# pbluc/avrecode-ms

Measured on AMD Instinct MI355X. Metric: H.264 bytes/s recompressed (CABAC re-encode of recorded bin streams, bit-exact vs CPU), higher is better.
Workload: dtype u32

## Files before the change

avrecode-ms_amd/csrc/avr_k1p.h:

```cpp
#pragma once
#include <stdint.h>

#include "avr_chunk.h"

#if defined(__HIPCC__)
#define AVR_HD __host__ __device__ inline
#else
#define AVR_HD inline
#endif

namespace avr {
namespace k1p {

#if defined(__HIP_DEVICE_COMPILE__)
#define AVR_PIN2(a, b) asm volatile("" : "+v"(a), "+v"(b))
#else
#define AVR_PIN2(a, b) ((void)0)
#endif

constexpr uint32_t kNone = 0xffffffffu;
constexpr uint32_t kMaxStretch = 16 * kChunk;
constexpr uint32_t kCodeBypass = 252;
constexpr uint32_t kCodePad = 252;

struct alignas(16) U4 { uint32_t x, y, z, w; };

AVR_HD int clz32(uint32_t x) {
#if defined(__HIP_DEVICE_COMPILE__)
    return __clz(x);
#else
    return x ? __builtin_clz(x) : 32;
#endif
}

AVR_HD uint32_t code_sym(uint32_t c) { return ((c >> 1) ^ c) & 1u; }
AVR_HD bool code_is_bypass(uint32_t c) { return (c >> 1) == 126u; }
AVR_HD bool code_is_boundary(uint32_t c) { return code_sym(c) && !code_is_bypass(c); }
AVR_HD uint32_t code_terminate(uint32_t b) { return 255u - b; }
AVR_HD uint32_t code_context(uint32_t s, uint32_t bin) { return s >= 126 ? 255u - ((bin ^ s) & 1u) : (s << 1) | bin; }

AVR_HD uint32_t post_lps_range(uint32_t row, uint32_t q, uint32_t *shift) {
    const uint32_t rl = (row >> (8 * q)) & 0xffu;
    const uint32_t sh = uint32_t(clz32(rl)) - 23;
    *shift = sh;
    return rl << sh;
}

struct CodeEntry { uint32_t row, meta; };
AVR_HD CodeEntry code_entry(uint32_t c, const uint32_t *rows ) {
    if (code_is_bypass(c)) return CodeEntry{0u, 0x100u | ((c & 1u) << 1)};
    return CodeEntry{rows[c >> 2], code_sym(c) * 3u};
}

AVR_HD int clz32_nz(uint32_t x) { return __builtin_clz(x); }
AVR_HD uint32_t lps_range(uint32_t row, uint32_t R) {
#if defined(__HIP_DEVICE_COMPILE__)
    return __builtin_amdgcn_perm(row, 0u, R >> 6);
#else
    return (row >> ((R >> 3) & 24)) & 0xffu;
#endif
}
AVR_HD uint32_t mul24(uint32_t a, uint32_t b) {
#if defined(__HIP_DEVICE_COMPILE__)
    return __umul24(a, b);
#else
    return a * b;
#endif
}
AVR_HD uint32_t step_range(const CodeEntry &e, uint32_t *R) {
    const uint32_t rl = lps_range(e.row, *R);
    const uint32_t rm = *R - rl;
    const uint32_t x = (e.meta & 1u) ? rl : rm;
    const uint32_t sh = uint32_t(clz32_nz(x)) - 23;
    *R = x << sh;
    return sh + (e.meta >> 8);
}

struct alignas(16) CodeEntryC { uint32_t row, side, k, adj; };
AVR_HD CodeEntryC code_entry_c(const CodeEntry &e) {
    const uint32_t sym = e.meta & 1u, adds = (e.meta >> 1) & 1u, byp = e.meta >> 8;
    return CodeEntryC{e.row, sym ? ~0u : 0u, adds ? (byp ? 1u : 2u) : 0u, byp - 23u};
}
AVR_HD uint32_t step_range_c(const CodeEntryC &e, uint32_t *R, uint32_t *v) {
    const uint32_t rl = lps_range(e.row, *R);
    const uint32_t rm = *R - rl;
    const uint32_t x = (rl & e.side) | (rm & ~e.side);
    const uint32_t lz = uint32_t(clz32_nz(x));
    *v = mul24(rm, e.k);
    *R = x << (lz - 23);
    return lz + e.adj;
}


struct Stretch {
    uint32_t first;
    uint32_t end;
    uint32_t t_exit[4];
    uint16_t r_exit[4];
    uint8_t exit_q;
    uint8_t too_long;
    uint8_t pad[2];
};

struct LinearCodes {
    const uint8_t *p;
    AVR_HD U4 load16(uint32_t i) const { return *reinterpret_cast<const U4 *>(p + i); }
    AVR_HD uint32_t byte(uint32_t i) const { return p[i]; }
};

template <class Src, class F>
AVR_HD void for_codes_in(const Src &src, uint32_t from, uint32_t n, F &&f) {
    for (uint32_t base = from & ~15u; base < n; base += 16) {
        const U4 v = src.load16(base);
        uint32_t w0 = v.x, w1 = v.y, w2 = v.z, w3 = v.w;
#if defined(__HIP_DEVICE_COMPILE__)
#pragma unroll 1
#endif
        for (uint32_t k = 0; k < 4; k++) {
            const uint32_t d = w0;
            w0 = w1; w1 = w2; w2 = w3;
            const uint32_t i = base + 4 * k;
            if (i + 0 - from < n - from && f(i + 0, d & 0xffu)) return;
            if (i + 1 - from < n - from && f(i + 1, (d >> 8) & 0xffu)) return;
            if (i + 2 - from < n - from && f(i + 2, (d >> 16) & 0xffu)) return;
            if (i + 3 - from < n - from && f(i + 3, d >> 24)) return;
        }
    }
}
template <class F>
AVR_HD void for_codes(const uint8_t *res, uint32_t from, uint32_t n, F &&f) { for_codes_in(LinearCodes{res}, from, n, f); }

template <class G, class G4>
AVR_HD void for_codes_all(const uint8_t *res, uint32_t from, uint32_t to, G &&g, G4 &&g4) {
    if (from >= to) return;
    auto group16 = [&](const U4 &v) {
        uint32_t w0 = v.x, w1 = v.y, w2 = v.z, w3 = v.w;
#if defined(__HIP_DEVICE_COMPILE__)
#pragma unroll 1
#endif
        for (uint32_t k = 0; k < 4; k++) {
            const uint32_t d = w0;
            w0 = w1; w1 = w2; w2 = w3;
            g4(d);
        }
    };
    const uint32_t head_end = ((from + 15) & ~15u) < to ? ((from + 15) & ~15u) : to;
    for_codes(res, from, head_end, [&](uint32_t, uint32_t c) { g(c); return false; });
    uint32_t base = head_end;
    for (; (base & 63) && base + 16 <= to; base += 16) group16(*reinterpret_cast<const U4 *>(res + base));
    if (base + 64 <= to) {
        const U4 *p = reinterpret_cast<const U4 *>(res + base);
        U4 v0 = p[0], v1 = p[1], v2 = p[2], v3 = p[3];
        for (; base + 64 <= to; base += 64) {
            const U4 *q = reinterpret_cast<const U4 *>(res + (base + 128 <= to ? base + 64 : base));
            const U4 n0 = q[0], n1 = q[1], n2 = q[2], n3 = q[3];
            group16(v0); group16(v1); group16(v2); group16(v3);
            v0 = n0; v1 = n1; v2 = n2; v3 = n3;
        }
    }
    for (; base + 16 <= to; base += 16) group16(*reinterpret_cast<const U4 *>(res + base));
    if (base < to) for_codes(res, base, to, [&](uint32_t, uint32_t c) { g(c); return false; });
}

AVR_HD void code_entries4(const CodeEntry *codes, uint32_t d, CodeEntry e[4]) {
    e[0] = codes[d & 0xffu]; e[1] = codes[(d >> 8) & 0xffu]; e[2] = codes[(d >> 16) & 0xffu]; e[3] = codes[d >> 24];
    AVR_PIN2(e[0].row, e[0].meta); AVR_PIN2(e[1].row, e[1].meta); AVR_PIN2(e[2].row, e[2].meta); AVR_PIN2(e[3].row, e[3].meta);
}
AVR_HD void code_entries4(const CodeEntryC *codes, uint32_t d, CodeEntryC e[4]) {
    e[0] = codes[d & 0xffu]; e[1] = codes[(d >> 8) & 0xffu]; e[2] = codes[(d >> 16) & 0xffu]; e[3] = codes[d >> 24];
    AVR_PIN2(e[0].row, e[0].side); AVR_PIN2(e[1].row, e[1].side); AVR_PIN2(e[2].row, e[2].side); AVR_PIN2(e[3].row, e[3].side);
}

AVR_HD void b1_stretch(const uint8_t *res, uint32_t n, uint32_t chunk, const CodeEntry *codes, uint32_t max_stretch,
                       Stretch *o) {
    const uint32_t lo = chunk_start(chunk), limit = chunk_start(chunk + 1);
    uint32_t R[4], T[4] = {0, 0, 0, 0};
    uint32_t i;
    o->too_long = 0;
    o->exit_q = 0;
    o->pad[0] = o->pad[1] = 0;
    if (chunk == 0) {
        o->first = 0;
        R[0] = R[1] = R[2] = R[3] = 510;
        i = 0;
    } else {
// ... 237 lines not shown
```

avrecode-ms_amd/csrc/avr_k1p.hip:

```cpp
#include <hip/hip_runtime.h>

#include <mutex>
#include <stdint.h>
#include <stdlib.h>
#include <type_traits>

#include "avr_coder.h"
#include "avr_internal.h"
#include "avr_k1p.h"
#include "avr_tables.h"

namespace avr {

static __device__ const CabacTables d_tables = make_cabac_tables();

using namespace k1p;

struct Plan {
    const uint16_t *recs;
    const uint64_t *rec_off;
    const uint32_t *n_bins;
    const uint64_t *res_off;
    const uint32_t *chunk_base, *chunk_slice;
    const uint32_t *blk_base, *blk_slice;
    const uint64_t *dig_off;
    uint32_t n_states;
    uint32_t ns_full;
    const uint16_t *table;
    const uint16_t *index;
    const uint8_t *recs8;
};
constexpr uint32_t kNotUsed = 0xffffu;

struct TileCodes {
    const uint8_t *base;
    uint32_t chunk0;
    __device__ __forceinline__ size_t at(uint32_t i) const {
        return group_at(chunk0 + chunk_of(i), bin_in_chunk(i) >> 4);
    }
    static __device__ __forceinline__ size_t group_at(uint32_t gc, uint32_t g) { return ((size_t(gc >> 6) * kChunkCodeGroups + g) * kTileChunks + (gc & 63u)) * 16; }
    __device__ __forceinline__ U4 load16(uint32_t i) const { return *reinterpret_cast<const U4 *>(base + at(i)); }
    __device__ __forceinline__ uint32_t byte(uint32_t i) const { return base[at(i) + (i & 15u)]; }
};


constexpr uint32_t kCensusBlocks = 32;
__global__ __launch_bounds__(256) void k_k1p_census(Plan p, uint32_t total_blocks, const int32_t *status, uint32_t *used, uint32_t stride) {
    __shared__ uint8_t flag[AVR_MAX_STATES];
    __shared__ uint32_t bm[32];
    for (uint32_t k = threadIdx.x; k < AVR_MAX_STATES / 4; k += 256) reinterpret_cast<uint32_t *>(flag)[k] = 0;
    if (threadIdx.x < 32) bm[threadIdx.x] = 0;
    __syncthreads();
    const uint32_t b = blockIdx.x * kCensusBlocks + (threadIdx.x >> 3), t = threadIdx.x & 7, nk = p.ns_full;
    if (b < total_blocks) {
        const uint32_t s = p.blk_slice[b];
        if (status[s] == AVR_SLICE_OK) {
            const uint32_t n = p.n_bins[s], i0 = (b - p.blk_base[s]) * kSortBlock;
            const uint32_t i1 = i0 + kSortBlock < n ? i0 + kSortBlock : n;
            const uint16_t *r = p.recs + p.rec_off[s];
            for (uint32_t l = b % stride; l < kSortBlock / 64; l += stride) {
                const uint32_t i = i0 + l * 64 + t * 8;
                if (i >= i1) continue;
                const uint4 v = *reinterpret_cast<const uint4 *>(r + i);
                const uint32_t w[4] = {v.x, v.y, v.z, v.w};
#pragma unroll
                for (uint32_t j = 0; j < 8; j++) {
                    const uint32_t sel = ((w[j >> 1] >> ((j & 1) * 16)) & 0xffffu) >> 1;
                    if (i + j < i1 && sel < nk) flag[sel] = 1;
                }
            }
        }
    }
    __syncthreads();
    {
        const uint32_t f = reinterpret_cast<const uint32_t *>(flag)[threadIdx.x];
        const uint32_t nib = (f & 1u) | ((f >> 7) & 2u) | ((f >> 14) & 4u) | ((f >> 21) & 8u);
        if (nib) atomicOr(&bm[threadIdx.x >> 3], nib << ((threadIdx.x & 7) * 4));
    }
    __syncthreads();
    if (threadIdx.x < 32) {
        const uint32_t mine = bm[threadIdx.x];
        if (mine & ~__hip_atomic_load(&used[threadIdx.x], __ATOMIC_RELAXED, __HIP_MEMORY_SCOPE_AGENT)) atomicOr(&used[threadIdx.x], mine);
    }
}

__global__ __launch_bounds__(256) void k_k1p_swap(int32_t *status, uint32_t n, int32_t a, int32_t b, int32_t c, int32_t d) {
    const uint32_t i = blockIdx.x * 256 + threadIdx.x;
    if (i >= n) return;
    const int32_t v = status[i];
    if (v == a) status[i] = b;
    else if (v == c) status[i] = d;
}

__global__ __launch_bounds__(AVR_MAX_STATES) void k_k1p_densemap(const uint32_t *used, uint16_t *table, uint16_t *index, uint32_t *n_dense) {
    __shared__ uint32_t sc[AVR_MAX_STATES];
    const uint32_t k = threadIdx.x;
    const uint32_t bit = (used[k >> 5] >> (k & 31)) & 1u;
    sc[k] = bit;
    __syncthreads();
    for (uint32_t d = 1; d < AVR_MAX_STATES; d <<= 1) {
        const uint32_t v = k >= d ? sc[k - d] : 0;
        __syncthreads();
        sc[k] += v;
        __syncthreads();
    }
    const uint32_t id = sc[k] - bit;
    table[k] = bit ? uint16_t(id) : uint16_t(kNotUsed);
    if (bit) index[id] = uint16_t(k);
    if (k >= sc[AVR_MAX_STATES - 1]) index[k] = uint16_t(kNotUsed);
    if (k == AVR_MAX_STATES - 1) *n_dense = sc[AVR_MAX_STATES - 1];
}

__global__ __launch_bounds__(256) void k_k1p_tn(uint8_t *tn) {
    const uint32_t i = blockIdx.x * 256 + threadIdx.x;
    if (i >= kTnBytes) return;
    const uint32_t n = 31 - __clz((i >> 7) + 1), j = i - ((128u << n) - 128u);
    uint32_t st = j >> n;
    for (uint32_t b = 0; b < n; b++) {
        const uint32_t nx = d_tables.packed[st][1], bin = (j >> b) & 1u;
        st = ((bin ^ st) & 1u) ? (nx >> 8) & 0xffu : nx & 0xffu;
    }
    tn[i] = uint8_t(st);
}

template <class F>
__device__ __forceinline__ void for_record_groups(const uint16_t *r, uint32_t i0, uint32_t i1, F &&f) {
    uint32_t i = i0;
    if (i + 32 <= i1) {
        const uint32_t last = i0 + ((i1 - i0) / 32u - 1u) * 32u;
        const U4 *q = reinterpret_cast<const U4 *>(r + i);
        U4 v0 = q[0], v1 = q[1], v2 = q[2], v3 = q[3];
        for (; i + 32 <= i1; i += 32) {
            const U4 *qn = reinterpret_cast<const U4 *>(r + (i + 32 <= last ? i + 32 : last));
            const U4 n0 = qn[0], n1 = qn[1], n2 = qn[2], n3 = qn[3];
            f(i, v0, std::false_type{}); f(i + 8, v1, std::false_type{}); f(i + 16, v2, std::false_type{}); f(i + 24, v3, std::false_type{});
            v0 = n0; v1 = n1; v2 = n2; v3 = n3;
        }
    }
    for (; i < i1; i += 8) f(i, *reinterpret_cast<const U4 *>(r + i), std::true_type{});
}

template <class F>
__device__ __forceinline__ void for_record_groups8(const uint8_t *r, uint32_t i0, uint32_t i1, F &&f) {
    uint32_t i = i0;
    if (i + 64 <= i1) {
        const uint32_t last = i0 + ((i1 - i0) / 64u - 1u) * 64u;
        const U4 *q = reinterpret_cast<const U4 *>(r + i);
        U4 v0 = q[0], v1 = q[1], v2 = q[2], v3 = q[3];
        for (; i + 64 <= i1; i += 64) {
            const U4 *qn = reinterpret_cast<const U4 *>(r + (i + 64 <= last ? i + 64 : last));
            const U4 n0 = qn[0], n1 = qn[1], n2 = qn[2], n3 = qn[3];
            f(i, v0, std::false_type{}); f(i + 16, v1, std::false_type{}); f(i + 32, v2, std::false_type{}); f(i + 48, v3, std::false_type{});
            v0 = n0; v1 = n1; v2 = n2; v3 = n3;
        }
    }
    for (; i < i1; i += 16) f(i, *reinterpret_cast<const U4 *>(r + i), std::true_type{});
}

template <class SelT, bool R8>
__global__ __launch_bounds__(512) void k_k1p_local(Plan p, uint32_t total_chunks, int32_t *status, uint32_t *lbits,
                                                   uint16_t *lend, uint32_t *n_retry) {
    extern __shared__ uint32_t local_lds[];
    constexpr uint32_t kSelTab = R8 ? 128 : 2048;
    __shared__ SelT sel_tab[kSelTab];
    const uint32_t nk = p.n_states, lane = threadIdx.x & 63, wv = threadIdx.x >> 6;
    const uint32_t cnt_rows = (nk + 5) / 2;
    const uint32_t wave_dwords = (kChunkBitDwords + 1 + cnt_rows) * 64;
    uint32_t *bits = local_lds + wv * wave_dwords;
    uint32_t *cnt = bits + (kChunkBitDwords + 1) * 64;
    for (uint32_t sel = threadIdx.x; sel < kSelTab; sel += blockDim.x) {
        uint32_t k;
        if (R8) k = sel < nk ? sel : sel == AVR_SEL8_TERMINATE ? nk : sel == AVR_SEL8_BYPASS ? nk + 1 : nk + 3;
        else if (sel < AVR_MAX_STATES) {
            const uint32_t d = p.table[sel];
            k = d < nk ? d : sel < p.ns_full ? nk + 2 : nk + 3;
        } else k = sel == AVR_SEL_TERMINATE ? nk : sel == AVR_SEL_BYPASS ? nk + 1 : nk + 3;
        sel_tab[sel] = SelT((k >> 1) * 256u | (k & 1u) * 16u);
    }
    for (uint32_t i = lane; i < wave_dwords; i += 64) bits[i] = 0;
    __syncthreads();
    const uint32_t gc0 = (blockIdx.x * (blockDim.x >> 6) + wv) * 64, gc = gc0 + lane;
    uint32_t i0 = 0, i1 = 0, n = 0, s = 0;
    bool mine = false;
    const uint16_t *r = p.recs;
    const uint8_t *r8 = p.recs8;
    uint32_t misaligned = 0;
    if (gc < total_chunks) {
        s = p.chunk_slice[gc];
        if (status[s] == AVR_SLICE_OK) {
            mine = true;
            n = p.n_bins[s];
            const ChunkSpan sp = chunk_span(gc - p.chunk_base[s], n);
            i1 = sp.i1; i0 = sp.i0 > i1 ? i1 : sp.i0;
            if (R8) {
                const uint64_t off = p.rec_off[s];
                misaligned = uint32_t(off & 15u);
                r8 = p.recs8 + (off & ~uint64_t(15));
            } else {
                r = p.recs + p.rec_off[s];
            }
        }
    }
    uint32_t *my_cnt = cnt + lane;
    uint32_t *my_bits = bits + lane;
    uint8_t *cnt_b = reinterpret_cast<uint8_t *>(my_cnt), *bits_b = reinterpret_cast<uint8_t *>(my_bits);
    auto for_groups = [&](auto &&f) { for_record_groups(r, i0, i1, f); };
    uint32_t high = 0;
    const uint32_t k_pad = nk + 1;
    const uint32_t e_pad = (k_pad >> 1) * 256u | (k_pad & 1u) * 16u;
    auto group8 = [&](uint32_t base, const U4 &v, auto masked, uint32_t e[16], uint32_t bin[16]) {
        const uint32_t w[4] = {v.x, v.y, v.z, v.w};
#pragma unroll
        for (uint32_t j = 0; j < 16; j++) {
            const uint32_t b = (w[j >> 2] >> (8 * (j & 3))) & 0xffu;
            e[j] = sel_tab[b >> 1];
            if (decltype(masked)::value) e[j] = base + j < i1 ? e[j] : e_pad;
            bin[j] = b & 1u;
        }
    };
    if (R8) for_record_groups8(r8, i0, i1, [&](uint32_t base, const U4 &v, auto masked) {
        uint32_t e[16], bin[16];
        group8(base, v, masked, e, bin);
#pragma unroll
        for (uint32_t j = 0; j < 16; j++)
            __hip_atomic_fetch_add(reinterpret_cast<uint32_t *>(cnt_b + (e[j] & ~255u)), 1u << (e[j] & 31u), __ATOMIC_RELAXED,
                                   __HIP_MEMORY_SCOPE_WORKGROUP);
    });
    else for_groups([&](uint32_t base, const U4 &v, auto masked) {
        const uint32_t w[4] = {v.x, v.y, v.z, v.w};
        high |= (w[0] | w[1]) | (w[2] | w[3]);
        uint32_t e[8];
#pragma unroll
        for (uint32_t j = 0; j < 8; j++) {
            e[j] = sel_tab[((w[j >> 1] >> ((j & 1) * 16)) >> 1) & 0x7ffu];
            if (decltype(masked)::value) e[j] = base + j < i1 ? e[j] : e_pad;
        }
#pragma unroll
        for (uint32_t j = 0; j < 8; j++)
            __hip_atomic_fetch_add(reinterpret_cast<uint32_t *>(cnt_b + (e[j] & ~255u)), 1u << (e[j] & 31u), __ATOMIC_RELAXED,
                                   __HIP_MEMORY_SCOPE_WORKGROUP);
    });
    auto count_of = [&](uint32_t k) { return (my_cnt[64 * (k >> 1)] >> (16 * (k & 1u))) & 0xffffu; };
    const uint32_t n_term = count_of(nk), n_missed = count_of(nk + 2), n_invalid = count_of(nk + 3) | (high & 0xf000f000u) | misaligned;
    uint32_t term_at = 0;
    {
        uint32_t run = 0;
        for (uint32_t j = 0; j < cnt_rows; j++) {
            const uint32_t c = my_cnt[64 * j], c0 = c & 0xffffu, c1 = c >> 16;
            const uint32_t s0 = 2 * j <= nk ? run : kChunk, s1 = 2 * j + 1 <= nk ? run + c0 : kChunk;
            if (2 * j == nk) term_at = s0;
            if (2 * j + 1 == nk) term_at = s1;
            my_cnt[64 * j] = s0 | s1 << 16;
            run += (2 * j <= nk ? c0 : 0u) + (2 * j + 1 <= nk ? c1 : 0u);
        }
    }
    if (R8) for_record_groups8(r8, i0, i1, [&](uint32_t base, const U4 &v, auto masked) {
        uint32_t e[16], bin[16], pos[16];
        group8(base, v, masked, e, bin);
#pragma unroll
        for (uint32_t j = 0; j < 16; j++)
            pos[j] = __hip_atomic_fetch_add(reinterpret_cast<uint32_t *>(cnt_b + (e[j] & ~255u)), 1u << (e[j] & 31u), __ATOMIC_RELAXED,
                                            __HIP_MEMORY_SCOPE_WORKGROUP);
#pragma unroll
        for (uint32_t j = 0; j < 16; j++) {
            const uint32_t at = (pos[j] >> (e[j] & 31u)) & kChunkPosMask;
            const uint32_t row = at >> 5 < kChunkBitDwords ? at >> 5 : kChunkSpareRow;
            __hip_atomic_fetch_or(reinterpret_cast<uint32_t *>(bits_b + row * 256u), bin[j] << (at & 31u), __ATOMIC_RELAXED,
                                  __HIP_MEMORY_SCOPE_WORKGROUP);
        }
    });
    else for_groups([&](uint32_t base, const U4 &v, auto masked) {
        const uint32_t w[4] = {v.x, v.y, v.z, v.w};
        uint32_t e[8], pos[8];
#pragma unroll
        for (uint32_t j = 0; j < 8; j++) {
            e[j] = sel_tab[((w[j >> 1] >> ((j & 1) * 16)) >> 1) & 0x7ffu];
            if (decltype(masked)::value) e[j] = base + j < i1 ? e[j] : e_pad;
        }
#pragma unroll
        for (uint32_t j = 0; j < 8; j++)
            pos[j] = __hip_atomic_fetch_add(reinterpret_cast<uint32_t *>(cnt_b + (e[j] & ~255u)), 1u << (e[j] & 31u), __ATOMIC_RELAXED,
                                            __HIP_MEMORY_SCOPE_WORKGROUP);
#pragma unroll
        for (uint32_t j = 0; j < 8; j++) {
            const uint32_t at = (pos[j] >> (e[j] & 31u)) & kChunkPosMask;
            const uint32_t row = at >> 5 < kChunkBitDwords ? at >> 5 : kChunkSpareRow;
            const uint32_t bin = (w[j >> 1] >> ((j & 1) * 16)) & 1u;
            __hip_atomic_fetch_or(reinterpret_cast<uint32_t *>(bits_b + row * 256u), bin << (at & 31u), __ATOMIC_RELAXED,
                                  __HIP_MEMORY_SCOPE_WORKGROUP);
        }
    });
    if (mine) {
        uint32_t ones = 0;
        for (uint32_t pos = term_at; pos < term_at + n_term;) {
            const uint32_t lo = pos & 31u, take = 32u - lo < term_at + n_term - pos ? 32u - lo : term_at + n_term - pos;
            const uint32_t mask = (take == 32u ? 0xffffffffu : (1u << take) - 1u) << lo;
            ones += __popc(my_bits[64 * (pos >> 5)] & mask);
            pos += take;
        }
        constexpr uint32_t kTerm1 = (AVR_SEL_TERMINATE << 1) | 1, kTerm1_8 = (AVR_SEL8_TERMINATE << 1) | 1;
        auto last_is_term1 = [&]() { return i1 == n && (R8 ? r8[misaligned + n - 1] == kTerm1_8 : r[n - 1] == kTerm1); };
        const bool bad_term = ones > 1u || (ones == 1u && !last_is_term1());
        if (n_invalid || bad_term) status[s] = AVR_SLICE_BAD_RECORD;
        else if (n_missed && atomicCAS(&status[s], AVR_SLICE_OK, AVR_SLICE_RETRY_CENSUS) == AVR_SLICE_OK) atomicAdd(n_retry, 1u);
    }
    {
        uint32_t *dst = lbits + size_t(gc0) * kChunkBitDwords;
        const uint32_t lim = gc0 < total_chunks ? (total_chunks - gc0 < 64 ? total_chunks - gc0 : 64) * kChunkBitDwords : 0;
        for (uint32_t f = lane; f < lim; f += 64) dst[f] = bits[64 * (f % kChunkBitDwords) + f / kChunkBitDwords];
    }
    if (nk) {
        uint16_t *dst = lend + size_t(gc0) * nk;
        const uint32_t lim = gc0 < total_chunks ? (total_chunks - gc0 < 64 ? total_chunks - gc0 : 64) * nk : 0;
        uint32_t ch = lane / nk, k = lane - ch * nk;
        const uint32_t dch = 64 / nk, dk = 64 - dch * nk;
        for (uint32_t f = lane; f < lim; f += 64) {
            dst[f] = uint16_t(cnt[64 * (k >> 1) + ch] >> (16 * (k & 1u)));
            ch += dch; k += dk;
            if (k >= nk) { k -= nk; ch++; }
        }
    }
}

constexpr uint32_t kChainLanes = 22, kChainWaves = 8;
__device__ __forceinline__ uint4 window(const uint32_t *bw, uint32_t pos) {
    const uint32_t wi = (pos >> 5) & (kChunkBitDwords - 1);
    return make_uint4(bw[wi], bw[wi + 1], bw[wi + 2], bw[wi + 3]);
}
__global__ __launch_bounds__(64 * kChainWaves) void k_k1p_ctxchain(Plan p, uint32_t n_slices, uint32_t groups, uint32_t chain_lanes, const int32_t *status,
                                                      const uint8_t *tng, const uint32_t *lbits, const uint16_t *lend,
                                                      const uint8_t *init_states, uint8_t *est, uint8_t *final_states) {
    __shared__ uint8_t tn[kTnBytes];
    for (uint32_t i = threadIdx.x; i < kTnBytes / 16; i += 64 * kChainWaves) reinterpret_cast<uint4 *>(tn)[i] = reinterpret_cast<const uint4 *>(tng)[i];
    __syncthreads();
    const uint32_t wave = blockIdx.x * kChainWaves + (threadIdx.x >> 6), lane = threadIdx.x & 63;
    const uint32_t nk = p.n_states, pair = wave * 64 + lane;
    const uint32_t s = groups ? wave / groups : pair / nk, k = groups ? (wave - s * groups) + lane * groups : pair - s * nk;
    if ((groups && lane >= chain_lanes) || s >= n_slices || status[s] != AVR_SLICE_OK || k >= nk) return;
    const uint32_t col = p.index ? p.index[k] : k, row4 = ((nk + 3) >> 2) << 2;
    if (col >= p.ns_full) return;
    uint32_t st = init_states[size_t(s) * p.ns_full + col] & 127u;
    const uint32_t c0 = p.chunk_base[s], nc = chunks_of(p.n_bins[s]);
    const uint16_t *le = lend + size_t(c0) * nk + k;
    const uint32_t *bw_ahead = lbits + size_t(c0) * kChunkBitDwords;
    const uint32_t *bw_cur = bw_ahead;
    uint8_t *eo = est + size_t(c0) * row4 + k;
    auto ends = [&]() {
        const uint32_t e1 = le[0], em = le[-1];
        le += nk;
        return make_uint2(k ? em : 0u, e1);
    };
    uint2 e0 = ends(), e1 = ends(), e2 = ends(), e3 = ends();
    uint4 w0 = window(bw_ahead, e0.x), w1 = window(bw_ahead + kChunkBitDwords, e1.x);
    bw_ahead += 2 * kChunkBitDwords;
    for (uint32_t c = 0; c < nc; c++) {
        const uint2 e4 = ends();
        const uint4 w2 = window(bw_ahead, e2.x);
        bw_ahead += kChunkBitDwords;
        *eo = uint8_t(st);
        eo += row4;
        uint32_t pos = e0.x;
        const uint32_t end = e0.y;
        uint32_t left = (end > pos && st < 126) ? end - pos : 0u;
        const uint32_t sh = pos & 31u;
        auto four = [&](uint32_t avail) {
#pragma unroll
            for (uint32_t i = 0; i < 4; i++) {
                if (i && !__any(left != 0)) break;
                const uint32_t n = left < 8u ? left : 8u;
                uint32_t off = (128u << n) - 128u + (avail & ((1u << n) - 1u));
                asm volatile("" : "+v"(off));
                st = tn[(st << n) + off];
                avail >>= 8;
                left -= n;
            }
        };
        four(__builtin_amdgcn_alignbit(w0.y, w0.x, sh));
        if (__any(left != 0)) {
            four(__builtin_amdgcn_alignbit(w0.z, w0.y, sh));
            if (__any(left != 0)) {
                pos += 64;
                uint32_t avail = __builtin_amdgcn_alignbit(w0.w, w0.z, sh);
                uint32_t have = 32;
                while (left) {
                    if (have == 0) {
                        const uint4 win = window(bw_cur, pos);
                        avail = __builtin_amdgcn_alignbit(win.y, win.x, pos & 31u);
                        have = 32;
                    }
                    const uint32_t n = left < 8u ? left : 8u;
                    uint32_t off = (128u << n) - 128u + (avail & ((1u << n) - 1u));
                    asm volatile("" : "+v"(off));
                    st = tn[(st << n) + off];
                    avail >>= 8;
                    left -= n; pos += n; have -= 8;
                }
            }
        }
        bw_cur += kChunkBitDwords;
        e0 = e1; e1 = e2; e2 = e3; e3 = e4;
        w0 = w1; w1 = w2;
    }
    if (final_states) final_states[size_t(s) * p.ns_full + col] = uint8_t(st);
}

constexpr uint32_t kSegWaves = 16;
constexpr uint32_t kChainWaveSlots = 8192;

template <int NS>
__device__ __forceinline__ void chain_step(const uint8_t *tn, const uint32_t *bw_cur, uint32_t pos, uint32_t end, const uint4 &w0, uint32_t (&st)[NS]) {
    uint32_t left = end > pos ? end - pos : 0u;
    const uint32_t sh = pos & 31u;
    auto four = [&](uint32_t avail) {
#pragma unroll
        for (uint32_t i = 0; i < 4; i++) {
            if (i && !__any(left != 0)) break;
            const uint32_t n = left < 8u ? left : 8u;
            uint32_t off = (128u << n) - 128u + (avail & ((1u << n) - 1u));
            asm volatile("" : "+v"(off));
#pragma unroll
            for (int q = 0; q < NS; q++) st[q] = tn[(st[q] << n) + off];
            avail >>= 8;
            left -= n;
        }
    };
    four(__builtin_amdgcn_alignbit(w0.y, w0.x, sh));
    if (__any(left != 0)) {
        four(__builtin_amdgcn_alignbit(w0.z, w0.y, sh));
        if (__any(left != 0)) {
            pos += 64;
            uint32_t avail = __builtin_amdgcn_alignbit(w0.w, w0.z, sh);
            uint32_t have = 32;
            while (left) {
                if (have == 0) {
                    const uint32_t wi = (pos >> 5) & (kChunkBitDwords - 1);
                    avail = __builtin_amdgcn_alignbit(bw_cur[wi + 1], bw_cur[wi], pos & 31u);
                    have = 32;
                }
                const uint32_t n = left < 8u ? left : 8u;
                uint32_t off = (128u << n) - 128u + (avail & ((1u << n) - 1u));
                asm volatile("" : "+v"(off));
#pragma unroll
                for (int q = 0; q < NS; q++) st[q] = tn[(st[q] << n) + off];
                avail >>= 8;
                left -= n; pos += n; have -= 8;
            }
        }
    }
}

struct ChainLane { uint32_t s, k, seg, c_begin, c_end, nc, col; };
__device__ __forceinline__ bool chain_lane(const Plan &p, uint32_t n_slices, uint32_t n_segs, const int32_t *status, ChainLane *o) {
    const uint32_t wave = blockIdx.x * kSegWaves + (threadIdx.x >> 6), lane = threadIdx.x & 63, nk = p.n_states;
    const uint32_t seg = wave % n_segs, pair = (wave / n_segs) * 64 + lane;
    const uint32_t s = pair / nk, k = pair - s * nk;
    if (s >= n_slices || status[s] != AVR_SLICE_OK) return false;
    const uint32_t col = p.index ? p.index[k] : k;
    if (col >= p.ns_full) return false;
    const uint32_t nc = chunks_of(p.n_bins[s]), seg_len = (nc + n_segs - 1) / n_segs;
    const uint32_t c_begin = seg * seg_len < nc ? seg * seg_len : nc, c_end = c_begin + seg_len < nc ? c_begin + seg_len : nc;
    *o = ChainLane{s, k, seg, c_begin, c_end, nc, col};
    return true;
}

__global__ __launch_bounds__(64 * kSegWaves) void k_k1p_chain_seg(Plan p, uint32_t n_slices, uint32_t n_segs, const int32_t *status,
                                                       const uint8_t *tng, const uint32_t *lbits, const uint16_t *lend, uint8_t *est, SegSummary *summ) {
    __shared__ uint8_t tn[kTnBytes];
    for (uint32_t i = threadIdx.x; i < kTnBytes / 16; i += 64 * kSegWaves) reinterpret_cast<uint4 *>(tn)[i] = reinterpret_cast<const uint4 *>(tng)[i];
    __syncthreads();
    ChainLane L;
    if (!chain_lane(p, n_slices, n_segs, status, &L)) return;
    const uint32_t nk = p.n_states, row4 = ((nk + 3) >> 2) << 2, k = L.k;
    const uint32_t c0 = p.chunk_base[L.s] + L.c_begin, n_ch = L.c_end - L.c_begin;
    const uint16_t *le = lend + size_t(c0) * nk + k;
    const uint32_t *bw_ahead = lbits + size_t(c0) * kChunkBitDwords, *bw_cur = bw_ahead;
    uint8_t *eo = est + size_t(c0) * row4 + k;
    auto ends = [&]() { const uint32_t e1 = le[0], em = le[-1]; le += nk; return make_uint2(k ? em : 0u, e1); };
    uint2 e0 = ends(), e1 = ends(), e2 = ends(), e3 = ends();
    uint4 w0 = window(bw_ahead, e0.x), w1 = window(bw_ahead + kChunkBitDwords, e1.x);
    bw_ahead += 2 * kChunkBitDwords;
    uint32_t st[2] = {124u, 125u};
    uint32_t met_chunk = n_ch, n_bins = 0;
    uint64_t bits0 = 0, bits1 = 0;
    for (uint32_t c = 0; c < n_ch; c++) {
        const uint2 e4 = ends();
        const uint4 w2 = window(bw_ahead, e2.x);
        bw_ahead += kChunkBitDwords;
        if (st[0] == st[1]) {
            *eo = uint8_t(st[0]);
            met_chunk = met_chunk < c ? met_chunk : c;
        }
        eo += row4;
        const uint32_t pos = e0.x, end = e0.y, cnt = end > pos ? end - pos : 0u;
        if (n_bins < kSegBits && cnt) {
            const uint32_t sh = pos & 31u;
            const uint64_t lo = uint64_t(__builtin_amdgcn_alignbit(w0.y, w0.x, sh)) | uint64_t(__builtin_amdgcn_alignbit(w0.z, w0.y, sh)) << 32;
            const uint64_t got = cnt < 64u ? lo & ((uint64_t(1) << cnt) - 1) : lo;
            if (n_bins < 64u) { bits0 |= got << n_bins; bits1 |= n_bins ? got >> (64u - n_bins) : 0u; }
            else bits1 |= got << (n_bins - 64u);
        }
        n_bins += cnt > 64u ? kSegBits + 1u : cnt;
        chain_step<2>(tn, bw_cur, pos, end, w0, st);
        bw_cur += kChunkBitDwords;
        e0 = e1; e1 = e2; e2 = e3; e3 = e4;
        w0 = w1; w1 = w2;
    }
    SegSummary o;
    o.bits[0] = bits0; o.bits[1] = bits1; o.n_bins = n_bins; o.exit_state = uint8_t(st[0]); o.met = st[0] == st[1] && met_chunk < 0xffffu;
    o.met_chunk = uint16_t(met_chunk < 0xffffu ? met_chunk : 0xffffu);
    summ[(size_t(L.s) * nk + k) * n_segs + L.seg] = o;
}

template <bool NOTE>
__device__ __forceinline__ uint32_t chain_chunks(const uint8_t *tn, const uint32_t *lbits, const uint16_t *lend, uint8_t *est, uint32_t nk, uint32_t row4,
                                                 uint32_t k, uint32_t c_first, uint32_t n_ch, uint32_t st0) {
    const uint16_t *le = lend + size_t(c_first) * nk + k;
    const uint32_t *bw_ahead = lbits + size_t(c_first) * kChunkBitDwords, *bw_cur = bw_ahead;
    uint8_t *eo = est + size_t(c_first) * row4 + k;
    auto ends = [&]() { const uint32_t e1 = le[0], em = le[-1]; le += nk; return make_uint2(k ? em : 0u, e1); };
    uint2 e0 = ends(), e1 = ends(), e2 = ends(), e3 = ends();
    uint4 w0 = window(bw_ahead, e0.x), w1 = window(bw_ahead + kChunkBitDwords, e1.x);
    bw_ahead += 2 * kChunkBitDwords;
    uint32_t st[1] = {st0};
    for (uint32_t c = 0; c < n_ch; c++) {
        const uint2 e4 = ends();
        const uint4 w2 = window(bw_ahead, e2.x);
        bw_ahead += kChunkBitDwords;
        if (NOTE) { *eo = uint8_t(st[0]); eo += row4; }
        if (st[0] < 126u) chain_step<1>(tn, bw_cur, e0.x, e0.y, w0, st);
        bw_cur += kChunkBitDwords;
        e0 = e1; e1 = e2; e2 = e3; e3 = e4;
        w0 = w1; w1 = w2;
    }
    return st[0];
}

__global__ __launch_bounds__(64 * kSegWaves) void k_k1p_chain_fix(Plan p, uint32_t n_slices, uint32_t n_segs, const int32_t *status,
                                                       const uint8_t *tng, const uint32_t *lbits, const uint16_t *lend, const uint8_t *init_states,
                                                       uint8_t *est, const SegSummary *summ, uint8_t *final_states, uint32_t force_walk_every) {
    __shared__ uint8_t tn[kTnBytes];
    for (uint32_t i = threadIdx.x; i < kTnBytes / 16; i += 64 * kSegWaves) reinterpret_cast<uint4 *>(tn)[i] = reinterpret_cast<const uint4 *>(tng)[i];
    __syncthreads();
    ChainLane L;
    if (!chain_lane(p, n_slices, n_segs, status, &L)) return;
    const uint32_t nk = p.n_states, row4 = ((nk + 3) >> 2) << 2, k = L.k;
    const SegSummary *mine = summ + (size_t(L.s) * nk + k) * n_segs;
    const uint32_t init = init_states[size_t(L.s) * p.ns_full + L.col] & 127u;
    const uint32_t c_slice = p.chunk_base[L.s], seg_len = (L.nc + n_segs - 1) / n_segs;
    const bool distrust = force_walk_every && (L.s * nk + k) % force_walk_every == 0;
    uint32_t from = L.seg, entry = init;
    if (init < 126u) {
        while (from > 0 && (distrust || !mine[from - 1].met)) from--;
        if (from > 0) entry = mine[from - 1].exit_state;
        for (uint32_t g = from; g < L.seg; g++) {
            const SegSummary sg = mine[g];
            if (sg.n_bins <= kSegBits && !distrust) {
                uint64_t b = sg.bits[0], b_hi = sg.bits[1];
                for (uint32_t left = sg.n_bins; left;) {
                    const uint32_t n = left < 8u ? left : 8u;
                    entry = tn[(128u << n) - 128u + (entry << n) + (uint32_t(b) & ((1u << n) - 1u))];
                    b = (b >> 8) | (b_hi << 56); b_hi >>= 8; left -= n;
                }
            } else {
                const uint32_t g_begin = g * seg_len < L.nc ? g * seg_len : L.nc, g_end = g_begin + seg_len < L.nc ? g_begin + seg_len : L.nc;
                entry = chain_chunks<false>(tn, lbits, lend, est, nk, row4, k, c_slice + g_begin, g_end - g_begin, entry);
            }
        }
    }
    const SegSummary me = mine[L.seg];
    const uint32_t n_ch = L.c_end - L.c_begin;
    const bool met = me.met && init < 126u && !distrust;
    const uint32_t stop = met && me.met_chunk < n_ch ? me.met_chunk : n_ch;
    const uint32_t exit_state = chain_chunks<true>(tn, lbits, lend, est, nk, row4, k, c_slice + L.c_begin, stop, entry);
    if (final_states && (L.c_end == L.nc) && (L.c_begin < L.nc || L.seg == 0))
        final_states[size_t(L.s) * p.ns_full + L.col] = uint8_t(stop < n_ch ? me.exit_state : exit_state);
}

__device__ __forceinline__ CodeEntry device_code_entry(uint32_t c);
__device__ __forceinline__ uint2 device_codes2(uint32_t c);

constexpr uint32_t kStBypass = 128, kStTerminate = 129, kStPad = 130, kStNone = 131, kReplayStates = 132;

typedef uint16_t u16x2 __attribute__((ext_vector_type(2)));
__device__ __forceinline__ uint32_t pk_sub(uint32_t a, uint32_t b) { return __builtin_bit_cast(uint32_t, __builtin_bit_cast(u16x2, a) - __builtin_bit_cast(u16x2, b)); }
__device__ __forceinline__ uint32_t pk_add(uint32_t a, uint32_t b) { return __builtin_bit_cast(uint32_t, __builtin_bit_cast(u16x2, a) + __builtin_bit_cast(u16x2, b)); }
__device__ __forceinline__ uint32_t pk_shl(uint32_t a, uint32_t b) { return __builtin_bit_cast(uint32_t, __builtin_bit_cast(u16x2, a) << __builtin_bit_cast(u16x2, b)); }
__device__ __forceinline__ uint32_t pk_shr8(uint32_t a) { return (a >> 8) & 0x00ff00ffu; }
__device__ __forceinline__ uint32_t step_pair(uint32_t &Rp, uint32_t row, uint32_t rown, uint32_t shrow, bool sym, uint32_t extra) {
    const uint32_t sel = ((Rp >> 6) & 0x00030003u) | 0x0c000c00u;
    const uint32_t rl = __builtin_amdgcn_perm(row, row, sel);
    const uint32_t rm = pk_sub(Rp, rl);
    const uint32_t shm = pk_shr8(rm) ^ 0x00010001u;
    const uint32_t rn = __builtin_amdgcn_perm(rown, rown, sel) | 0x01000100u;
    const uint32_t shl = __builtin_amdgcn_perm(shrow, shrow, sel);
    Rp = sym ? rn : pk_shl(rm, shm);
    return (sym ? shl : shm) + extra;
}

struct B1Walk {
    uint32_t i0, i1, limit, n, max_stretch;
    const uint2 *codes2;
    uint32_t mode, Rp0, Rp1, Tp0, Tp1, T[4], Rm, Tm, end;
    bool merged;
    Stretch o;

    __device__ __forceinline__ void init(uint32_t chunk, uint32_t i0_, uint32_t i1_, uint32_t n_, uint32_t max_stretch_, const uint2 *codes2_) {
        i0 = i0_; i1 = i1_; limit = i0_ + kChunk; n = n_; max_stretch = max_stretch_; codes2 = codes2_;
        mode = 0; Rp0 = Rp1 = 0x01fe01feu; Tp0 = Tp1 = 0; T[0] = T[1] = T[2] = T[3] = 0; Rm = 510; Tm = 0; end = 0;
        merged = false;
        o.first = kNone; o.end = 0; o.exit_q = 0; o.too_long = 0; o.pad[0] = o.pad[1] = 0;
        for (int q = 0; q < 4; q++) { o.t_exit[q] = 0; o.r_exit[q] = 0; }
        if (chunk == 0) { o.first = 0; mode = 2; merged = true; }
    }
    __device__ __forceinline__ void flush_t() {
        T[0] += Tp0 & 0xffffu; T[1] += Tp0 >> 16; T[2] += Tp1 & 0xffffu; T[3] += Tp1 >> 16;
        Tp0 = Tp1 = 0;
    }
    __device__ __forceinline__ bool met() const { return Rp0 == Rp1 && (Rp0 >> 16) == (Rp0 & 0xffffu); }
    __device__ __forceinline__ void one(uint32_t idx, const uint4 &e) {
        const CodeEntry ce{e.x, e.y >> 16};
        const bool boundary = ce.meta & 1u;
        if (mode == 0) {
            if (idx < i1 && boundary) {
                o.first = idx;
                const uint32_t rown = codes2[(e.y >> 8) & 0xffu].x;
                Rp0 = __builtin_amdgcn_perm(rown, rown, 0x0c010c00u) | 0x01000100u;
                Rp1 = __builtin_amdgcn_perm(rown, rown, 0x0c030c02u) | 0x01000100u;
                mode = 1;
            }
        } else if (mode == 1) {
            const bool closing = idx >= limit && boundary;
            if (closing)
                o.exit_q |= uint8_t(((Rp0 >> 6) & 3u) | ((Rp0 >> 22) & 3u) << 2 | ((Rp1 >> 6) & 3u) << 4 | ((Rp1 >> 22) & 3u) << 6);
            const uint2 e2 = codes2[(e.y >> 8) & 0xffu];
            const uint32_t extra = (ce.meta >> 8) * 0x00010001u;
            Tp0 = pk_add(Tp0, step_pair(Rp0, ce.row, e2.x, e2.y, boundary, extra));
            Tp1 = pk_add(Tp1, step_pair(Rp1, ce.row, e2.x, e2.y, boundary, extra));
            if (closing) { end = idx + 1; mode = 3; }
            else if (met()) { Rm = Rp0 & 0xffffu; mode = 2; merged = true; }
        } else if (mode == 2) {
            const bool closing = idx >= limit && boundary;
            if (closing) o.exit_q = uint8_t(((Rm >> 6) & 3) * 0x55u);
            Tm += step_merged(e);
            if (closing) { end = idx + 1; mode = 3; }
            else if (idx >= limit && idx - i0 > max_stretch) { o.too_long = 1; end = idx + 1; mode = 3; }
        }
    }
    __device__ __forceinline__ uint32_t step_merged(const uint4 &e) {
        uint32_t v;
        return step_range_c(CodeEntryC{e.x, e.z, 0u, e.w}, &Rm, &v);
    }
    __device__ __forceinline__ void group(uint32_t base, const uint4 e[8]) {
        if (mode == 2 && base + 8 <= i1) {
#pragma unroll
            for (uint32_t j = 0; j < 8; j++) Tm += step_merged(e[j]);
        } else if (mode == 1 && base + 8 <= i1) {
#pragma unroll
            for (uint32_t j = 0; j < 8; j++) {
                const uint2 e2 = codes2[(e[j].y >> 8) & 0xffu];
                const bool sym = (e[j].y >> 16) & 1u;
                const uint32_t extra = (e[j].y >> 24) * 0x00010001u;
                Tp0 = pk_add(Tp0, step_pair(Rp0, e[j].x, e2.x, e2.y, sym, extra));
                Tp1 = pk_add(Tp1, step_pair(Rp1, e[j].x, e2.x, e2.y, sym, extra));
            }
            flush_t();
            if (met()) { Rm = Rp0 & 0xffffu; mode = 2; merged = true; }
        } else if (mode != 3) {
            for (uint32_t j = 0; j < 8; j++) if (base + j < n) one(base + j, e[j]);
            flush_t();
        }
    }
    __device__ __forceinline__ void chunk_done() { if (mode == 0) mode = 3; }
    __device__ __forceinline__ void tail(uint32_t base, const uint4 e[8]) {
        for (uint32_t j = 0; j < 8; j++) if (base + j < n && mode != 3) one(base + j, e[j]);
        flush_t();
    }
    __device__ __forceinline__ const Stretch &finish() {
        if (o.first != kNone) {
            o.end = mode != 3 ? n : end;
            for (uint32_t q = 0; q < 4; q++) {
                const uint32_t rq = ((q & 2u) ? Rp1 : Rp0) >> (16 * (q & 1u)) & 0xffffu;
                o.t_exit[q] = T[q] + (merged ? Tm : 0u);
                o.r_exit[q] = uint16_t(merged ? Rm : rq);
            }
        }
        return o;
// ... 815 lines not shown
```

Baseline: 24.88 billion.

## Restructure context-chain walk: remainder-first table step and 4-way unrolled lookahead ring

Replaces the per-chunk chain stepping with a chain_step that first consumes the leftover (count mod 8) bits through one variable-width table lookup, then whole bytes through the 8-bit section, with wave-uniform early exits. The chunk lookahead (end offsets and bit windows) moves into a ChainAhead ring that is unrolled four chunks at a time, so the register rotation each chunk disappears. In the segment kernel, bit-capture work is skipped once the chains meet and is guarded by a wave-level any test. This aims to cut ALU work and register shuffling in the serial state-machine walk, at the cost of more complex control flow and higher code size and register use.

```diff
diff --git a/avrecode-ms_amd/csrc/avr_k1p.h b/avrecode-ms_amd/csrc/avr_k1p.h
--- a/avrecode-ms_amd/csrc/avr_k1p.h
+++ b/avrecode-ms_amd/csrc/avr_k1p.h
@@ -31,6 +31,67 @@
 #else
     return x ? __builtin_clz(x) : 32;
 #endif
+}
+
+#if defined(__HIP_DEVICE_COMPILE__)
+#define AVR_ANY(x) __any(x)
+#define AVR_PIN1(a) asm volatile("" : "+v"(a))
+#else
+#define AVR_ANY(x) (x)
+#define AVR_PIN1(a) ((void)0)
+#endif
+AVR_HD constexpr uint32_t tn_section(uint32_t n) { return (128u << n) - 128u; }
+AVR_HD uint8_t tn_entry(uint32_t i, const uint32_t (*packed)[2]) {
+    const uint32_t n = 31u - uint32_t(clz32((i >> 7) + 1)), j = i - tn_section(n);
+    uint32_t st = j >> n;
+    for (uint32_t b = 0; b < n; b++) {
+        const uint32_t nx = packed[st][1], bin = (j >> b) & 1u;
+        st = ((bin ^ st) & 1u) ? (nx >> 8) & 0xffu : nx & 0xffu;
+    }
+    return uint8_t(st);
+}
+AVR_HD U4 chain_window(const uint32_t *bw, uint32_t pos) {
+    const uint32_t wi = (pos >> 5) & (kChunkBitDwords - 1);
+    return U4{bw[wi], bw[wi + 1], bw[wi + 2], bw[wi + 3]};
+}
+AVR_HD uint32_t funnel(uint32_t hi, uint32_t lo, uint32_t sh) {
+#if defined(__HIP_DEVICE_COMPILE__)
+    return __builtin_amdgcn_alignbit(hi, lo, sh);
+#else
+    return sh ? (lo >> sh) | (hi << (32u - sh)) : lo;
+#endif
+}
+template <int NS, int COUNT>
+AVR_HD bool chain_bytes(const uint8_t *tn, uint32_t avail, uint32_t first, uint32_t whole, uint32_t (&st)[NS]) {
+#pragma unroll
+    for (int i = 0; i < COUNT; i++) {
+        if (i && !AVR_ANY(whole > first + i)) return false;
+        if (whole > first + i) {
+            const uint32_t byte = (avail >> (8 * i)) & 0xffu;
+#pragma unroll
+            for (int q = 0; q < NS; q++) st[q] = tn[tn_section(8) + (st[q] << 8 | byte)];
+        }
+    }
+    return AVR_ANY(whole > first + COUNT);
+}
+template <int NS>
+AVR_HD void chain_step(const uint8_t *tn, const uint32_t *bw, uint32_t pos, uint32_t left, const U4 &w, uint32_t (&st)[NS]) {
+    const uint32_t sh = pos & 31u, rem = left & 7u, whole = left >> 3;
+    const uint32_t b0 = funnel(w.y, w.x, sh);
+    uint32_t off = tn_section(rem) + (b0 & ((1u << rem) - 1u));
+    AVR_PIN1(off);
+#pragma unroll
+    for (int q = 0; q < NS; q++) st[q] = tn[(st[q] << rem) + off];
+    if (!AVR_ANY(whole != 0)) return;
+    const uint32_t b1 = funnel(w.z, w.y, sh);
+    if (!chain_bytes<NS, 4>(tn, funnel(b1, b0, rem), 0, whole, st)) return;
+    const uint32_t b2 = funnel(w.w, w.z, sh);
+    if (!chain_bytes<NS, 4>(tn, funnel(b2, b1, rem), 4, whole, st)) return;
+    if (!chain_bytes<NS, 3>(tn, b2 >> rem, 8, whole, st)) return;
+    for (uint32_t first = 11;; first += 4) {
+        const uint32_t at = pos + rem + 8 * first, wi = (at >> 5) & (kChunkBitDwords - 1);
+        if (!chain_bytes<NS, 4>(tn, funnel(bw[wi + 1], bw[wi], at & 31u), first, whole, st)) return;
+    }
 }
 
 AVR_HD uint32_t code_sym(uint32_t c) { return ((c >> 1) ^ c) & 1u; }
diff --git a/avrecode-ms_amd/csrc/avr_k1p.hip b/avrecode-ms_amd/csrc/avr_k1p.hip
--- a/avrecode-ms_amd/csrc/avr_k1p.hip
+++ b/avrecode-ms_amd/csrc/avr_k1p.hip
@@ -114,13 +114,7 @@
 __global__ __launch_bounds__(256) void k_k1p_tn(uint8_t *tn) {
     const uint32_t i = blockIdx.x * 256 + threadIdx.x;
     if (i >= kTnBytes) return;
-    const uint32_t n = 31 - __clz((i >> 7) + 1), j = i - ((128u << n) - 128u);
-    uint32_t st = j >> n;
-    for (uint32_t b = 0; b < n; b++) {
-        const uint32_t nx = d_tables.packed[st][1], bin = (j >> b) & 1u;
-        st = ((bin ^ st) & 1u) ? (nx >> 8) & 0xffu : nx & 0xffu;
-    }
-    tn[i] = uint8_t(st);
+    tn[i] = tn_entry(i, d_tables.packed);
 }
 
 template <class F>
@@ -323,10 +317,43 @@
 }
 
 constexpr uint32_t kChainLanes = 22, kChainWaves = 8;
-__device__ __forceinline__ uint4 window(const uint32_t *bw, uint32_t pos) {
-    const uint32_t wi = (pos >> 5) & (kChunkBitDwords - 1);
-    return make_uint4(bw[wi], bw[wi + 1], bw[wi + 2], bw[wi + 3]);
-}
+struct ChainAhead {
+    const uint16_t *le;
+    const uint32_t *bw_ahead, *bw_cur;
+    uint32_t nk, k;
+    uint2 e[4];
+    U4 w[2];
+    __device__ __forceinline__ uint2 ends() {
+        const uint32_t e1 = le[0], em = le[-1];
+        le += nk;
+        return make_uint2(k ? em : 0u, e1);
+    }
+    __device__ __forceinline__ ChainAhead(const uint32_t *lbits, const uint16_t *lend, uint32_t nk_, uint32_t k_, uint32_t c_first)
+        : le(lend + size_t(c_first) * nk_ + k_), bw_ahead(lbits + size_t(c_first) * kChunkBitDwords), bw_cur(bw_ahead), nk(nk_), k(k_) {
+        for (int j = 0; j < 4; j++) e[j] = ends();
+        for (int j = 0; j < 2; j++) { w[j] = chain_window(bw_ahead, e[j].x); bw_ahead += kChunkBitDwords; }
+    }
+    struct Chunk { uint32_t pos, cnt; U4 w; const uint32_t *bw; };
+    template <int J>
+    __device__ __forceinline__ Chunk take() {
+        const Chunk c{e[J].x, e[J].y > e[J].x ? e[J].y - e[J].x : 0u, w[J & 1], bw_cur};
+        e[J] = ends();
+        w[J & 1] = chain_window(bw_ahead, e[(J + 2) & 3].x);
+        bw_ahead += kChunkBitDwords;
+        bw_cur += kChunkBitDwords;
+        return c;
+    }
+    template <class F>
+    __device__ __forceinline__ void walk(uint32_t n_ch, F &&f) {
+        uint32_t c = 0;
+        for (; c + 4 <= n_ch; c += 4) { f(take<0>()); f(take<1>()); f(take<2>()); f(take<3>()); }
+        for (; c < n_ch; c++) {
+            f(take<0>());
+            const uint2 t = e[0]; e[0] = e[1]; e[1] = e[2]; e[2] = e[3]; e[3] = t;
+            const U4 u = w[0]; w[0] = w[1]; w[1] = u;
+        }
+    }
+};
 __global__ __launch_bounds__(64 * kChainWaves) void k_k1p_ctxchain(Plan p, uint32_t n_slices, uint32_t groups, uint32_t chain_lanes, const int32_t *status,
                                                       const uint8_t *tng, const uint32_t *lbits, const uint16_t *lend,
                                                       const uint8_t *init_states, uint8_t *est, uint8_t *final_states) {
@@ -339,115 +366,20 @@
     if ((groups && lane >= chain_lanes) || s >= n_slices || status[s] != AVR_SLICE_OK || k >= nk) return;
     const uint32_t col = p.index ? p.index[k] : k, row4 = ((nk + 3) >> 2) << 2;
     if (col >= p.ns_full) return;
-    uint32_t st = init_states[size_t(s) * p.ns_full + col] & 127u;
+    uint32_t st[1] = {init_states[size_t(s) * p.ns_full + col] & 127u};
     const uint32_t c0 = p.chunk_base[s], nc = chunks_of(p.n_bins[s]);
-    const uint16_t *le = lend + size_t(c0) * nk + k;
-    const uint32_t *bw_ahead = lbits + size_t(c0) * kChunkBitDwords;
-    const uint32_t *bw_cur = bw_ahead;
     uint8_t *eo = est + size_t(c0) * row4 + k;
-    auto ends = [&]() {
-        const uint32_t e1 = le[0], em = le[-1];
-        le += nk;
-        return make_uint2(k ? em : 0u, e1);
-    };
-    uint2 e0 = ends(), e1 = ends(), e2 = ends(), e3 = ends();
-    uint4 w0 = window(bw_ahead, e0.x), w1 = window(bw_ahead + kChunkBitDwords, e1.x);
-    bw_ahead += 2 * kChunkBitDwords;
-    for (uint32_t c = 0; c < nc; c++) {
-        const uint2 e4 = ends();
-        const uint4 w2 = window(bw_ahead, e2.x);
-        bw_ahead += kChunkBitDwords;
-        *eo = uint8_t(st);
+    ChainAhead ahead(lbits, lend, nk, k, c0);
+    ahead.walk(nc, [&](const ChainAhead::Chunk &c) {
+        *eo = uint8_t(st[0]);
         eo += row4;
-        uint32_t pos = e0.x;
-        const uint32_t end = e0.y;
-        uint32_t left = (end > pos && st < 126) ? end - pos : 0u;
-        const uint32_t sh = pos & 31u;
-        auto four = [&](uint32_t avail) {
-#pragma unroll
-            for (uint32_t i = 0; i < 4; i++) {
-                if (i && !__any(left != 0)) break;
-                const uint32_t n = left < 8u ? left : 8u;
-                uint32_t off = (128u << n) - 128u + (avail & ((1u << n) - 1u));
-                asm volatile("" : "+v"(off));
-                st = tn[(st << n) + off];
-                avail >>= 8;
-                left -= n;
-            }
-        };
-        four(__builtin_amdgcn_alignbit(w0.y, w0.x, sh));
-        if (__any(left != 0)) {
-            four(__builtin_amdgcn_alignbit(w0.z, w0.y, sh));
-            if (__any(left != 0)) {
-                pos += 64;
-                uint32_t avail = __builtin_amdgcn_alignbit(w0.w, w0.z, sh);
-                uint32_t have = 32;
-                while (left) {
-                    if (have == 0) {
-                        const uint4 win = window(bw_cur, pos);
-                        avail = __builtin_amdgcn_alignbit(win.y, win.x, pos & 31u);
-                        have = 32;
-                    }
-                    const uint32_t n = left < 8u ? left : 8u;
-                    uint32_t off = (128u << n) - 128u + (avail & ((1u << n) - 1u));
-                    asm volatile("" : "+v"(off));
-                    st = tn[(st << n) + off];
-                    avail >>= 8;
-                    left -= n; pos += n; have -= 8;
-                }
-            }
-        }
-        bw_cur += kChunkBitDwords;
-        e0 = e1; e1 = e2; e2 = e3; e3 = e4;
-        w0 = w1; w1 = w2;
-    }
-    if (final_states) final_states[size_t(s) * p.ns_full + col] = uint8_t(st);
+        chain_step<1>(tn, c.bw, c.pos, st[0] < 126u ? c.cnt : 0u, c.w, st);
+    });
+    if (final_states) final_states[size_t(s) * p.ns_full + col] = uint8_t(st[0]);
 }
 
 constexpr uint32_t kSegWaves = 16;
 constexpr uint32_t kChainWaveSlots = 8192;
-
-template <int NS>
-__device__ __forceinline__ void chain_step(const uint8_t *tn, const uint32_t *bw_cur, uint32_t pos, uint32_t end, const uint4 &w0, uint32_t (&st)[NS]) {
-    uint32_t left = end > pos ? end - pos : 0u;
-    const uint32_t sh = pos & 31u;
-    auto four = [&](uint32_t avail) {
-#pragma unroll
-        for (uint32_t i = 0; i < 4; i++) {
-            if (i && !__any(left != 0)) break;
-            const uint32_t n = left < 8u ? left : 8u;
-            uint32_t off = (128u << n) - 128u + (avail & ((1u << n) - 1u));
-            asm volatile("" : "+v"(off));
-#pragma unroll
-            for (int q = 0; q < NS; q++) st[q] = tn[(st[q] << n) + off];
-            avail >>= 8;
-            left -= n;
-        }
-    };
-    four(__builtin_amdgcn_alignbit(w0.y, w0.x, sh));
-    if (__any(left != 0)) {
-        four(__builtin_amdgcn_alignbit(w0.z, w0.y, sh));
-        if (__any(left != 0)) {
-            pos += 64;
-            uint32_t avail = __builtin_amdgcn_alignbit(w0.w, w0.z, sh);
-            uint32_t have = 32;
-            while (left) {
-                if (have == 0) {
-                    const uint32_t wi = (pos >> 5) & (kChunkBitDwords - 1);
-                    avail = __builtin_amdgcn_alignbit(bw_cur[wi + 1], bw_cur[wi], pos & 31u);
-                    have = 32;
-                }
-                const uint32_t n = left < 8u ? left : 8u;
-                uint32_t off = (128u << n) - 128u + (avail & ((1u << n) - 1u));
-                asm volatile("" : "+v"(off));
-#pragma unroll
-                for (int q = 0; q < NS; q++) st[q] = tn[(st[q] << n) + off];
-                avail >>= 8;
-                left -= n; pos += n; have -= 8;
-            }
-        }
-    }
-}
 
 struct ChainLane { uint32_t s, k, seg, c_begin, c_end, nc, col; };
 __device__ __forceinline__ bool chain_lane(const Plan &p, uint32_t n_slices, uint32_t n_segs, const int32_t *status, ChainLane *o) {
@@ -472,39 +404,31 @@
     if (!chain_lane(p, n_slices, n_segs, status, &L)) return;
     const uint32_t nk = p.n_states, row4 = ((nk + 3) >> 2) << 2, k = L.k;
     const uint32_t c0 = p.chunk_base[L.s] + L.c_begin, n_ch = L.c_end - L.c_begin;
-    const uint16_t *le = lend + size_t(c0) * nk + k;
-    const uint32_t *bw_ahead = lbits + size_t(c0) * kChunkBitDwords, *bw_cur = bw_ahead;
     uint8_t *eo = est + size_t(c0) * row4 + k;
-    auto ends = [&]() { const uint32_t e1 = le[0], em = le[-1]; le += nk; return make_uint2(k ? em : 0u, e1); };
-    uint2 e0 = ends(), e1 = ends(), e2 = ends(), e3 = ends();
-    uint4 w0 = window(bw_ahead, e0.x), w1 = window(bw_ahead + kChunkBitDwords, e1.x);
-    bw_ahead += 2 * kChunkBitDwords;
     uint32_t st[2] = {124u, 125u};
-    uint32_t met_chunk = n_ch, n_bins = 0;
+    uint32_t met_chunk = n_ch, n_bins = 0, at = 0;
     uint64_t bits0 = 0, bits1 = 0;
-    for (uint32_t c = 0; c < n_ch; c++) {
-        const uint2 e4 = ends();
-        const uint4 w2 = window(bw_ahead, e2.x);
-        bw_ahead += kChunkBitDwords;
+    ChainAhead ahead(lbits, lend, nk, k, c0);
+    ahead.walk(n_ch, [&](const ChainAhead::Chunk &c) {
         if (st[0] == st[1]) {
             *eo = uint8_t(st[0]);
-            met_chunk = met_chunk < c ? met_chunk : c;
+            met_chunk = met_chunk < at ? met_chunk : at;
+            if (at < 0xffffu) n_bins = kSegBits + 1u;
         }
         eo += row4;
-        const uint32_t pos = e0.x, end = e0.y, cnt = end > pos ? end - pos : 0u;
-        if (n_bins < kSegBits && cnt) {
-            const uint32_t sh = pos & 31u;
-            const uint64_t lo = uint64_t(__builtin_amdgcn_alignbit(w0.y, w0.x, sh)) | uint64_t(__builtin_amdgcn_alignbit(w0.z, w0.y, sh)) << 32;
+        at++;
+        const uint32_t cnt = c.cnt;
+        const bool room = n_bins < kSegBits && cnt;
+        if (__any(room) && room) {
+            const uint32_t sh = c.pos & 31u;
+            const uint64_t lo = uint64_t(__builtin_amdgcn_alignbit(c.w.y, c.w.x, sh)) | uint64_t(__builtin_amdgcn_alignbit(c.w.z, c.w.y, sh)) << 32;
             const uint64_t got = cnt < 64u ? lo & ((uint64_t(1) << cnt) - 1) : lo;
             if (n_bins < 64u) { bits0 |= got << n_bins; bits1 |= n_bins ? got >> (64u - n_bins) : 0u; }
             else bits1 |= got << (n_bins - 64u);
         }
         n_bins += cnt > 64u ? kSegBits + 1u : cnt;
-        chain_step<2>(tn, bw_cur, pos, end, w0, st);
-        bw_cur += kChunkBitDwords;
-        e0 = e1; e1 = e2; e2 = e3; e3 = e4;
-        w0 = w1; w1 = w2;
-    }
+        chain_step<2>(tn, c.bw, c.pos, cnt, c.w, st);
+    });
     SegSummary o;
     o.bits[0] = bits0; o.bits[1] = bits1; o.n_bins = n_bins; o.exit_state = uint8_t(st[0]); o.met = st[0] == st[1] && met_chunk < 0xffffu;
     o.met_chunk = uint16_t(met_chunk < 0xffffu ? met_chunk : 0xffffu);
@@ -514,24 +438,13 @@
 template <bool NOTE>
 __device__ __forceinline__ uint32_t chain_chunks(const uint8_t *tn, const uint32_t *lbits, const uint16_t *lend, uint8_t *est, uint32_t nk, uint32_t row4,
                                                  uint32_t k, uint32_t c_first, uint32_t n_ch, uint32_t st0) {
-    const uint16_t *le = lend + size_t(c_first) * nk + k;
-    const uint32_t *bw_ahead = lbits + size_t(c_first) * kChunkBitDwords, *bw_cur = bw_ahead;
     uint8_t *eo = est + size_t(c_first) * row4 + k;
-    auto ends = [&]() { const uint32_t e1 = le[0], em = le[-1]; le += nk; return make_uint2(k ? em : 0u, e1); };
-    uint2 e0 = ends(), e1 = ends(), e2 = ends(), e3 = ends();
-    uint4 w0 = window(bw_ahead, e0.x), w1 = window(bw_ahead + kChunkBitDwords, e1.x);
-    bw_ahead += 2 * kChunkBitDwords;
     uint32_t st[1] = {st0};
-    for (uint32_t c = 0; c < n_ch; c++) {
-        const uint2 e4 = ends();
-        const uint4 w2 = window(bw_ahead, e2.x);
-        bw_ahead += kChunkBitDwords;
+    ChainAhead ahead(lbits, lend, nk, k, c_first);
+    ahead.walk(n_ch, [&](const ChainAhead::Chunk &c) {
         if (NOTE) { *eo = uint8_t(st[0]); eo += row4; }
-        if (st[0] < 126u) chain_step<1>(tn, bw_cur, e0.x, e0.y, w0, st);
-        bw_cur += kChunkBitDwords;
-        e0 = e1; e1 = e2; e2 = e3; e3 = e4;
-        w0 = w1; w1 = w2;
-    }
+        chain_step<1>(tn, c.bw, c.pos, st[0] < 126u ? c.cnt : 0u, c.w, st);
+    });
     return st[0];
 }
 
```

Measured after the change: 25.72 billion (median of 6 runs). 1.03x the previous value.
